# Ecogenomics/CheckM

Hardware: NVIDIA H100
Metric: genomes/hour (higher is better)
Workload: dtype int16 (SSV) / u8 (MSV) / int16 (Viterbi) / f32 (Forward, domain definition)

## Files before the change

checkm_b200/csrc/fwdback_blk.cuh:

```cuda
#pragma once
#include "device_utils.cuh"
#include "engine.hpp"
#include "fwdback.cuh"

namespace ckm {

constexpr int BLK_LOOKAHEAD_MAXQ = 16;

template <int Q, bool TSMEM>
struct BlkModel {
  int M;
  const float *rfb;
  const float4 *tsm;
  float4 t0[TSMEM ? 1 : Q], t1[TSMEM ? 1 : Q];
  int lane;
  __device__ __forceinline__ float4 T0(int q) const { return TSMEM ? tsm[q * 32 + lane] : t0[TSMEM ? 0 : q]; }
  __device__ __forceinline__ float4 T1(int q) const { return TSMEM ? tsm[(Q + q) * 32 + lane] : t1[TSMEM ? 0 : q]; }
};

template <int Q, bool TSMEM>
__device__ __forceinline__ void blk_model_load(BlkModel<Q, TSMEM> &bm, const ModelScalars &ms, const float4 *tfb, const float *rfb,
                                               float4 *tsm, int lane) {
  bm.M = ms.M; bm.lane = lane;
  bm.rfb = rfb + ms.blk_off * 32 * KPAD + lane;
  bm.tsm = tsm;
  const float4 *src = tfb + ms.blk_off * 32 * 2;
  if (TSMEM) {
    __syncwarp();
    for (int q = 0; q < Q; ++q) { tsm[q * 32 + lane] = __ldg(src + (q * 32 + lane) * 2); tsm[(Q + q) * 32 + lane] = __ldg(src + (q * 32 + lane) * 2 + 1); }
    __syncwarp();
  } else {
#pragma unroll
    for (int q = 0; q < Q; ++q) { bm.t0[TSMEM ? 0 : q] = __ldg(src + (q * 32 + lane) * 2); bm.t1[TSMEM ? 0 : q] = __ldg(src + (q * 32 + lane) * 2 + 1); }
  }
}

template <int Q, bool TSMEM, bool FULL, bool STORE_D = true>
__device__ __forceinline__ float forward_blk(const BlkModel<Q, TSMEM> &bm, const uint8_t *__restrict__ res, int L, const Specials sp,
                                             float *xmx, float *full) {
  const int lane = bm.lane;
  float Mx[Q], Ix[Q], Dx[Q];
#pragma unroll
  for (int q = 0; q < Q; ++q) { Mx[q] = 0.0f; Ix[q] = 0.0f; Dx[q] = 0.0f; }
  if (FULL) {
#pragma unroll
    for (int z = 0; z < 3 * Q; ++z) full[z * 32 + lane] = 0.0f;
  }
  float xE = 0.0f, xN = 1.0f, xJ = 0.0f, xB = sp.nmove, xC = 0.0f, totscale = 0.0f;
  if (xmx != nullptr && lane == 0) { xmx[X_E] = xE; xmx[X_N] = xN; xmx[X_J] = xJ; xmx[X_B] = xB; xmx[X_C] = xC; xmx[X_SCALE] = 1.0f; }
  constexpr bool LA = (Q <= BLK_LOOKAHEAD_MAXQ);
  float ecur[Q];
  int xnext;
  if (LA) {
    const float *rp = bm.rfb + (size_t)((L >= 1) ? __ldg(res) : 0) * Q * 32;
#pragma unroll
    for (int q = 0; q < Q; ++q) ecur[q] = __ldg(rp + q * 32);
    xnext = (L >= 2) ? __ldg(res + 1) : 0;
  } else xnext = (L >= 1) ? __ldg(res) : 0;
  for (int i = 1; i <= L; ++i) {
    float enext[LA ? Q : 1];
    {
      const float *rp = bm.rfb + (size_t)xnext * Q * 32;
      if (LA) {
#pragma unroll
        for (int q = 0; q < Q; ++q) enext[LA ? q : 0] = __ldg(rp + q * 32);
        xnext = (i + 2 <= L) ? __ldg(res + i + 1) : 0;
      } else {
#pragma unroll
        for (int q = 0; q < Q; ++q) ecur[q] = __ldg(rp + q * 32);
        xnext = (i + 1 <= L) ? __ldg(res + i) : 0;
      }
    }
    float pm_in = __shfl_up_sync(0xffffffffu, Mx[Q - 1], 1), pi_in = __shfl_up_sync(0xffffffffu, Ix[Q - 1], 1), pd_in = __shfl_up_sync(0xffffffffu, Dx[Q - 1], 1);
    if (lane == 0) { pm_in = 0.0f; pi_in = 0.0f; pd_in = 0.0f; }
    float md[Q], esum = 0.0f;
#pragma unroll
    for (int q = Q - 1; q >= 0; --q) {
      const float4 t0 = bm.T0(q), t1 = bm.T1(q);
      const float pm = (q > 0) ? Mx[q - 1] : pm_in, pi = (q > 0) ? Ix[q - 1] : pi_in, pd = (q > 0) ? Dx[q - 1] : pd_in;
      float sv = xB * t0.x;
      sv += pm * t0.y;
      sv += pi * t0.z;
      sv += pd * t0.w;
      sv *= ecur[q];
      const float nI = Mx[q] * t1.y + Ix[q] * t1.z;
      md[q] = sv * t1.x;
      Mx[q] = sv; Ix[q] = nI;
      esum += sv;
    }
    float Bb = 0.0f, Tb = 1.0f;
#pragma unroll
    for (int q = 0; q < Q; ++q) { const float tdd = bm.T1(q).w; Bb = md[q] + Bb * tdd; Tb *= tdd; }
    float Bs = Bb, Ts = Tb;
#pragma unroll
    for (int o = 1; o < 32; o <<= 1) {
      const float Bl = __shfl_up_sync(0xffffffffu, Bs, o), Tl = __shfl_up_sync(0xffffffffu, Ts, o);
      if (lane >= o) { Bs = Bs + Bl * Ts; Ts = Ts * Tl; }
    }
    float d = __shfl_up_sync(0xffffffffu, Bs, 1);
    if (lane == 0) d = 0.0f;
#pragma unroll
    for (int q = 0; q < Q; ++q) {
// ... 5 lines not shown
    xE = warp_sum_float(esum);
    xN = xN * sp.nloop;
    xC = (xC * sp.nloop) + (xE * sp.emove);
    xJ = (xJ * sp.nloop) + (xE * sp.eloop);
    xB = (xJ * sp.nmove) + (xN * sp.nmove);
    float scale = 1.0f;
    if (xE > 1.0e4f) {
      scale = xE;
      const float inv = __fdiv_rn(1.0f, xE);
      xN = __fdiv_rn(xN, xE); xC = __fdiv_rn(xC, xE); xJ = __fdiv_rn(xJ, xE); xB = __fdiv_rn(xB, xE);
#pragma unroll
      for (int q = 0; q < Q; ++q) { Mx[q] *= inv; Dx[q] *= inv; Ix[q] *= inv; }
      totscale += (float)log((double)xE);
      xE = 1.0f;
    }
    if (FULL) {
      float *fr = full + (size_t)i * 3 * Q * 32 + lane;
#pragma unroll
      for (int q = 0; q < Q; ++q) { fr[q * 32] = Mx[q]; if (STORE_D) fr[(Q + q) * 32] = Dx[q]; fr[(2 * Q + q) * 32] = Ix[q]; }
    }
    if (xmx != nullptr && lane == 0) {
      float *xr = xmx + (size_t)i * X_NX;
      xr[X_E] = xE; xr[X_N] = xN; xr[X_J] = xJ; xr[X_B] = xB; xr[X_C] = xC; xr[X_SCALE] = scale;
    }
    if (LA) {
#pragma unroll
      for (int q = 0; q < Q; ++q) ecur[q] = enext[LA ? q : 0];
    }
  }
  return totscale + (float)log((double)(xC * sp.nmove));
}

__device__ __forceinline__ void prefetch_l2(const void *p) { asm volatile("prefetch.global.L2 [%0];" ::"l"(p)); }
template <int Q, bool TSMEM, int MODE>
__device__ __forceinline__ void backward_blk(const BlkModel<Q, TSMEM> &bm, const uint8_t *__restrict__ res, int L, const Specials sp,
                                             const float *fxmx, float *bxmx, float *full) {
  const int lane = bm.lane, M = bm.M;
  float Mx[Q], Ix[Q], Dx[Q];
#pragma unroll
  for (int q = 0; q < Q; ++q) { Mx[q] = 0.0f; Ix[q] = 0.0f; Dx[q] = 0.0f; }
  float xC = 0.0f, xE = 0.0f, xJ = 0.0f, xN = 0.0f, xB = 0.0f;
  constexpr bool LA = (Q <= BLK_LOOKAHEAD_MAXQ);
  float ecur[Q];
#pragma unroll
  for (int q = 0; q < Q; ++q) ecur[q] = 0.0f;
  int xnext = (L >= 1) ? __ldg(res + L - 1) : 0;
  for (int i = L; i >= 0; --i) {
    float enext[LA ? Q : 1];
    if (LA) {
      const float *rp = bm.rfb + (size_t)xnext * Q * 32;
#pragma unroll
      for (int q = 0; q < Q; ++q) enext[LA ? q : 0] = __ldg(rp + q * 32);
      xnext = (i >= 2) ? __ldg(res + i - 2) : 0;
    } else if (i < L) {
      const float *rp = bm.rfb + (size_t)xnext * Q * 32;
#pragma unroll
      for (int q = 0; q < Q; ++q) ecur[q] = __ldg(rp + q * 32);
      xnext = (i >= 1) ? __ldg(res + i - 1) : 0;
    }
    if (MODE == 2 && i >= 3) {
      const float *fr = full + (size_t)(i - 2) * 3 * Q * 32;
      if (lane < Q) { prefetch_l2(fr + lane * 32); prefetch_l2(fr + (2 * Q + lane) * 32); }
    }
    float em[Q];
    if (i == L) {
      xC = sp.nmove; xE = xC * sp.emove; xB = 0.0f; xJ = 0.0f; xN = 0.0f;
#pragma unroll
      for (int q = 0; q < Q; ++q) em[q] = 0.0f;
    } else {
      float part = 0.0f;
#pragma unroll
      for (int q = 0; q < Q; ++q) { em[q] = Mx[q] * ecur[q]; part += em[q] * bm.T0(q).x; }
      xB = warp_sum_float(part);
      xC = xC * sp.nloop;
      xJ = (xB * sp.nmove) + (xJ * sp.nloop);
      xN = (xB * sp.nmove) + (xN * sp.nloop);
      xE = (xC * sp.emove) + (xJ * sp.eloop);
    }
    const float s = (i >= 1) ? fxmx[(size_t)i * X_NX + X_SCALE] : 1.0f;
    if (i >= 1) {
      const float inv = (s > 1.0f) ? __fdiv_rn(1.0f, s) : 1.0f;
      float em_next = __shfl_down_sync(0xffffffffu, em[0], 1);
      float4 tn_next;
      {
        const float4 mine = bm.T0(0);
        tn_next.x = 0.0f;
        tn_next.y = __shfl_down_sync(0xffffffffu, mine.y, 1); tn_next.z = __shfl_down_sync(0xffffffffu, mine.z, 1); tn_next.w = __shfl_down_sync(0xffffffffu, mine.w, 1);
      }
      if (lane == 31) { em_next = 0.0f; tn_next.y = 0.0f; tn_next.z = 0.0f; tn_next.w = 0.0f; }
      float cb[Q];
// ... 70 lines not shown
```

checkm_b200/csrc/kernels_blk.cu:

```cuda
#include "engine.hpp"
#include "device_utils.cuh"
#include "stages.hpp"
#include "fwdback.cuh"
#include "fwdback_blk.cuh"
#include "domdef_common.cuh"
#include "filter_common.cuh"

namespace ckm {

constexpr int BLK_WARPS = 4;

__host__ __device__ constexpr size_t blk_tsm_bytes(int Q) { return (size_t)Q * 32 * 2 * sizeof(float4); }

template <int Q, bool TSMEM>
__global__ void __launch_bounds__(BLK_WARPS * 32) fwd2_kernel(FilterParams p) {
  extern __shared__ __align__(16) uint8_t bsm[];
  const int lane = threadIdx.x & 31, warp = threadIdx.x >> 5;
  float4 *tsm = reinterpret_cast<float4 *>(bsm) + (size_t)warp * Q * 32 * 2;
  const int n = min(*p.in_count, p.in_cap);
  for (int c = blockIdx.x * BLK_WARPS + warp; c < n; c += gridDim.x * BLK_WARPS) {
    Candidate cd = p.in[c];
    const ModelScalars ms = p.ms[cd.model];
    if (ms.vq != Q) continue;
    const int s = cd.seq, L = p.len[s];
    BlkModel<Q, TSMEM> bm;
    blk_model_load<Q, TSMEM>(bm, ms, p.tfb, p.rfb, tsm, lane);
    const float fsc = forward_blk<Q, TSMEM, false>(bm, p.res + p.off[s], L, make_specials(L, true), nullptr, nullptr);
    fwd_verdict(p, cd, fsc, ms, lane);
  }
}

template <int Q, bool TSMEM>
__global__ void __launch_bounds__(BLK_WARPS * 32) regions2_kernel(DomdefParams p) {
  extern __shared__ __align__(16) uint8_t bsm[];
  const int lane = threadIdx.x & 31, warp = threadIdx.x >> 5;
  float4 *tsm = reinterpret_cast<float4 *>(bsm) + (size_t)warp * Q * 32 * 2;
  for (int idx = p.pair_begin + blockIdx.x * BLK_WARPS + warp; idx < p.pair_end; idx += gridDim.x * BLK_WARPS) {
    const int pi = p.pair_order[idx];
    const PairWork pw = p.pairs[pi];
    const ModelScalars ms = p.ms[pw.model];
    if (ms.vq != Q) continue;
    const int L = pw.L;
    BlkModel<Q, TSMEM> bm;
    blk_model_load<Q, TSMEM>(bm, ms, p.tfb, p.rfb, tsm, lane);
    const uint8_t *res = p.res + p.off[pw.seq];
    const Specials sp = make_specials(L, true);
    float *xf = p.xf + pw.row_off * X_NX, *xb = p.xb + pw.row_off * X_NX;
    forward_blk<Q, TSMEM, false>(bm, res, L, sp, xf, nullptr);
    __syncwarp();
    backward_blk<Q, TSMEM, 0>(bm, res, L, sp, xf, xb, nullptr);
    __syncwarp();
    regions_tail(p, pi, L, sp, xf, xb, p.btot + pw.row_off, p.etot + pw.row_off, p.mocc + pw.row_off, p.n2sc + pw.row_off, lane);
    __syncwarp();
  }
}

template <int Q> struct BlockedLayout {
  const float *F; const float4 *tfb; int M;
  static __device__ __forceinline__ int at(int k) { return ((k - 1) % Q) * 32 + (k - 1) / Q; }
  __device__ __forceinline__ float cell(int row, int plane, int k) const { return F[((int64_t)row * 3 + plane) * (Q * 32) + at(k)]; }
  __device__ __forceinline__ float4 t0(int k) const { return __ldg(tfb + at(k) * 2); }
// ... 144 lines not shown
          if (lane >= o && Ps) { As = fmaxf(As, Al); Ps = (pl != 0); }
        }
        float d = __shfl_up_sync(0xffffffffu, As, 1);
        if (lane == 0) d = NINF;
#pragma unroll
        for (int q = 0; q < Q; ++q) {
          const bool in = (lane * Q + q + 1) <= M;
          oD[q] = in ? d : NINF;
          emax = fmaxf(emax, oD[q]);
          d = ps[q] ? fmaxf(a[q], d) : a[q];
        }
#pragma unroll
        for (int o = 16; o > 0; o >>= 1) emax = fmaxf(emax, __shfl_xor_sync(0xffffffffu, emax, o));
        os.row(sp, pps + r * 3, emax);
#pragma unroll
        for (int q = 0; q < Q; ++q) { orow[q * 32] = oM[q]; orow[(Q + q) * 32] = oD[q]; orow[(2 * Q + q) * 32] = oI[q]; }
        os.store(xo + (int64_t)r * X_NX, lane);
      }
      oasc = os.C;
    }
    __syncwarp();
    OaTrace tr;
    if (!range_err) tr = oa_traceback(BlockedLayout<Q>{Bm, p.tfb + ms.blk_off * 64, M}, p, pw, env, sp, xo, pps, Ld, M, lane);
    write_domain(p, env, n2sc, tr, envsc, oasc, lane);
    __syncwarp();
  }
}

template <class P, class KF>
static int launch_blk(KF kern, const char *name, int Q, bool tsmem, const P &p, int grid, size_t extra, cudaStream_t st) {
  return launch_kernel(kern, name, grid, BLK_WARPS * 32, (tsmem ? BLK_WARPS * blk_tsm_bytes(Q) : 0) + extra, st, p);
}
int launch_fwd2(const FilterParams &p, int cls, int grid, cudaStream_t st) {
  return with_class(cls, [&](auto Q, auto TSMEM) { return launch_blk(fwd2_kernel<Q, TSMEM>, "fwd2_kernel", Q, TSMEM, p, grid, 0, st); });
}
int launch_regions2(const DomdefParams &p, int cls, int grid, cudaStream_t st) {
  return with_class(cls, [&](auto Q, auto TSMEM) { return launch_blk(regions2_kernel<Q, TSMEM>, "regions2_kernel", Q, TSMEM, p, grid, 0, st); });
}
int launch_envelopes2(const DomdefParams &p, int cls, int grid, cudaStream_t st) {
  return with_class(cls, [&](auto Q, auto TSMEM) {
    return launch_blk(envelope2_kernel<Q, TSMEM>, "envelope2_kernel", Q, TSMEM, p, grid, BLK_WARPS * 32 * sizeof(float), st);
  });
}

}
```

checkm_b200/csrc/kernels_vitp.cu:

```cuda
#include "engine.hpp"
#include "device_utils.cuh"
#include "stages.hpp"
#include "filter_common.cuh"

namespace ckm {

constexpr uint32_t VP_FLOORW = 0xD800D800u;
constexpr int      VP_FLOOR  = -10240;
constexpr uint32_t VP_TFLOORW = 0xC000C000u;

__device__ __forceinline__ int vp_lo(uint32_t w) { return (int)(int16_t)(w & 0xffffu); }
__device__ __forceinline__ int vp_hi(uint32_t w) { return (int)w >> 16; }

__global__ void vit_count_kernel(FilterParams p, int32_t *cnt) {
  const int n = min(*p.in_count, p.in_cap);
  for (int i = blockIdx.x * blockDim.x + threadIdx.x; i < n; i += gridDim.x * blockDim.x) {
    const Candidate cd = p.in[i];
    if (!(cd.P > p.F2)) filter_pass(p, cd, 4);
    else if (p.ms[cd.model].vq == 0) vit_redo(p, cd);
    else atomicAdd(cnt + cd.model, 1);
  }
}

__global__ void __launch_bounds__(1024) vit_scan_kernel(FilterParams p, int32_t nmodels, const int32_t *cnt, int32_t *off, int32_t *choff) {
  __shared__ int ws[2][32];
  const int lane = threadIdx.x & 31, warp = threadIdx.x >> 5;
  int run_pairs = 0, run_chunks = 0;
  for (int c = 0; c < N_BLK_CLASSES; ++c) {
    if (threadIdx.x == 0) p.vit_cls_chunks[c] = run_chunks;
    for (int b = 0; b < nmodels; b += 1024) {
      const int m = b + threadIdx.x;
      const int v = (m < nmodels && blk_class(p.ms[m].vq) == c) ? cnt[m] : 0, h = (v + VITP_CHUNK - 1) / VITP_CHUNK;
      int sv = v, sh = h;
#pragma unroll
      for (int o = 1; o < 32; o <<= 1) {
        const int a = __shfl_up_sync(0xffffffffu, sv, o), d = __shfl_up_sync(0xffffffffu, sh, o);
        if (lane >= o) { sv += a; sh += d; }
      }
      if (lane == 31) { ws[0][warp] = sv; ws[1][warp] = sh; }
      __syncthreads();
      if (warp == 0) {
        int tv = ws[0][lane], th = ws[1][lane];
#pragma unroll
        for (int o = 1; o < 32; o <<= 1) {
          const int a = __shfl_up_sync(0xffffffffu, tv, o), d = __shfl_up_sync(0xffffffffu, th, o);
          if (lane >= o) { tv += a; th += d; }
        }
        ws[0][lane] = tv; ws[1][lane] = th;
      }
      __syncthreads();
      if (v > 0) {
        off[m] = run_pairs + (warp ? ws[0][warp - 1] : 0) + sv - v;
        choff[m] = run_chunks + (warp ? ws[1][warp - 1] : 0) + sh - h;
      }
      run_pairs += ws[0][31]; run_chunks += ws[1][31];
      __syncthreads();
    }
  }
  if (threadIdx.x == 0) p.vit_cls_chunks[N_BLK_CLASSES] = run_chunks;
}

__global__ void vit_scatter_kernel(FilterParams p, const int32_t *cnt, int32_t *fill, const int32_t *off, const int32_t *choff) {
  const int n = min(*p.in_count, p.in_cap);
  for (int i = blockIdx.x * blockDim.x + threadIdx.x; i < n; i += gridDim.x * blockDim.x) {
    const int m = p.in[i].model;
    if (!(p.in[i].P > p.F2) || p.ms[m].vq == 0) continue;
    const int r = atomicAdd(fill + m, 1), pos = off[m] + r;
    p.vit_idx[pos] = i;
    if (r % VITP_CHUNK == 0) p.vit_chunks[choff[m] + r / VITP_CHUNK] = make_int2(pos, off[m] + min(r + VITP_CHUNK, cnt[m]));
  }
}

int launch_vit_group(const FilterParams &p, int32_t nmodels, int32_t *ws, int grid, cudaStream_t st) {
  int32_t *cnt = ws, *fill = ws + nmodels, *off = ws + 2 * (size_t)nmodels, *choff = ws + 3 * (size_t)nmodels;
  cudaError_t e = cudaMemsetAsync(ws, 0, sizeof(int32_t) * 2 * (size_t)nmodels, st);
  if (e != cudaSuccess) return cuda_fail(e, "cudaMemsetAsync(vit groups)");
  vit_count_kernel<<<grid, 256, 0, st>>>(p, cnt);
  vit_scan_kernel<<<1, 1024, 0, st>>>(p, nmodels, cnt, off, choff);
  vit_scatter_kernel<<<grid, 256, 0, st>>>(p, cnt, fill, off, choff);
  e = cudaGetLastError();
  return e == cudaSuccess ? CKM_OK : cuda_fail(e, "vit grouping launch");
}

constexpr int VITP_THREADS = 128;

__host__ __device__ constexpr int vitp_smem_bytes(int W, bool tsmem) { return KPAD * W * 32 * 4 + (tsmem ? W * 64 * 16 : 0); }
__host__ __device__ constexpr int vitp_min_blocks(int W) { return W <= 4 ? 4 : (W <= 10 ? 3 : 2); }

template <int W, bool TSMEM>
__global__ void __launch_bounds__(VITP_THREADS, vitp_min_blocks(W)) vitp_kernel(FilterParams p, int cls) {
  extern __shared__ __align__(16) uint4 vsm[];
  __shared__ int s_chunk, s_next;
  __shared__ ModelScalars s_ms;
  uint32_t *esm = reinterpret_cast<uint32_t *>(vsm);
  uint4 *tws = vsm + KPAD * W * 8;
  const int lane = threadIdx.x & 31;
  const uint32_t sel = (lane == 0) ? 0x1054u : 0x3210u;
  const int c0 = p.vit_cls_chunks[cls], nch = p.vit_cls_chunks[cls + 1] - c0;
  for (;;) {
    __syncthreads();
    if (threadIdx.x == 0) {
      const int k = atomicAdd(p.vit_work + cls, 1);
      s_chunk = k;
      if (k < nch) {
        s_next = p.vit_chunks[c0 + k].x;
        s_ms = p.ms[p.in[p.vit_idx[s_next]].model];
      }
    }
    __syncthreads();
    const int k = s_chunk;
    if (k >= nch) break;
    const int2 ch = p.vit_chunks[c0 + k];
    const ModelScalars &ms = s_ms;
    {
      const uint4 *esrc = reinterpret_cast<const uint4 *>(p.rwp + ms.blk_off * 32 * (KPAD / 2));
      for (int z = threadIdx.x; z < KPAD * W * 8; z += VITP_THREADS) vsm[z] = __ldg(esrc + z);
      if (TSMEM) {
        const uint4 *tsrc = p.twp + ms.blk_off * 32;
        for (int z = threadIdx.x; z < W * 64; z += VITP_THREADS) tws[(z & 1) * (W * 32) + (z >> 1)] = __ldg(tsrc + z);
      }
    }
    uint4 tr0[TSMEM ? 1 : W], tr1[TSMEM ? 1 : W];
    if (!TSMEM) {
      const uint4 *tsrc = p.twp + ms.blk_off * 32;
#pragma unroll
      for (int w = 0; w < W; ++w) { tr0[TSMEM ? 0 : w] = __ldg(tsrc + (w * 32 + lane) * 2); tr1[TSMEM ? 0 : w] = __ldg(tsrc + (w * 32 + lane) * 2 + 1); }
    }
#define TR0(w) (TSMEM ? tws[(w) * 32 + lane] : tr0[TSMEM ? 0 : (w)])
#define TR1(w) (TSMEM ? tws[W * 32 + (w) * 32 + lane] : tr1[TSMEM ? 0 : (w)])
    __syncthreads();
    const uint32_t *erow = esm + lane;
    const int ddbound = ms.ddbound_w, cap = 32767 - (int)ms.vit_emax;
    const int e_move = ms.xw_e_move, e_loop = ms.xw_e_loop;
    for (;;) {
      int j = 0;
      if (lane == 0) j = atomicAdd(&s_next, 1);
      j = __shfl_sync(0xffffffffu, j, 0);
      if (j >= ch.y) break;
      const Candidate *cin = p.in + p.vit_idx[j];
      const int s = cin->seq, L = p.len[s];
      bool redo = false;
      const int tmove = p.tmove_w[s];
      const int cost = -tmove - (int)ms.vit_tbm + 64;
      const bool c1 = (cost - (int)ms.xw_e_loop <= 22528) && (cost <= 22240);
      const bool c1p = (cost - (int)ms.xw_e_loop <= 16384);
      redo = !c1;
      float vsc = 0.0f;
      if (!redo) {
        uint32_t Mx[W], Ix[W], Dx[W];
#pragma unroll
        for (int w = 0; w < W; ++w) { Mx[w] = VP_FLOORW; Ix[w] = VP_FLOORW; Dx[w] = VP_FLOORW; }
        int xN = ms.base_w, xB = xN + tmove, xJ = -32768, xC = -32768;
        const uint32_t *rp = reinterpret_cast<const uint32_t *>(p.res + p.off[s]);
        const int nw = (L + 3) >> 2;
        uint32_t wcur = (nw > 0) ? __ldg(rp) : 0u;
        bool stop = false;
        for (int q = 0; q < nw && !stop; ++q) {
          const uint32_t wnext = (q + 1 < nw) ? __ldg(rp + q + 1) : 0u;
#pragma unroll
          for (int rr = 0; rr < 4; ++rr) {
            if (q * 4 + rr >= L) { stop = true; break; }
            const uint32_t *ew = erow + ((wcur >> (8 * rr)) & 0xffu) * (W * 32);
            const uint32_t shM = __shfl_sync(0xffffffffu, Mx[W - 1], (lane + 31) & 31);
            const uint32_t shI = __shfl_sync(0xffffffffu, Ix[W - 1], (lane + 31) & 31);
            const uint32_t shD = __shfl_sync(0xffffffffu, Dx[W - 1], (lane + 31) & 31);
            const uint32_t pm0 = __byte_perm(shM, VP_FLOORW, sel), pi0 = __byte_perm(shI, VP_FLOORW, sel), pd0 = __byte_perm(shD, VP_FLOORW, sel);
            const uint32_t xBw = __byte_perm((uint32_t)xB, 0u, 0x1010u);
            uint32_t md[W];
            uint32_t xEw = VP_FLOORW, dmw = VP_FLOORW;
#pragma unroll
            for (int w = W - 1; w >= 0; --w) {
              const uint32_t pm = (w > 0) ? Mx[w - 1] : pm0, pi = (w > 0) ? Ix[w - 1] : pi0, pd = (w > 0) ? Dx[w - 1] : pd0;
// ... 83 lines not shown
```

checkm_b200/csrc/search.cu:

```cuda
#include <algorithm>
#include <atomic>
#include <chrono>
#include <cstdio>
#include <cmath>
#include <cstdlib>
#include <cstring>
#include <memory>
#include <vector>
#include "engine.hpp"
#include "stages.hpp"
#include "pool.hpp"

using namespace ckm;

namespace ckm {

std::atomic<int> g_live_engines{0};
thread_local ckm_engine *g_pool_engine = nullptr;
thread_local int g_pool_next = 0;
constexpr int X_NX_HOST = 6;
struct EnsembleJob;
int ensembles_launch(ckm_engine *e, const ckm_models *m, DomdefParams &p, const std::vector<PairWork> &pairs,
                     const std::vector<Region> &regs, const std::vector<int> &multi_idx, const std::vector<EnsembleCaps> &caps,
                     cudaStream_t st, EnsembleJob **job_out);
// ... 224 lines not shown
  for (int c = 0; c < 4; ++c) {
    if (gl[c].empty() || db->nseq == 0) continue;
    sp.group_list = s1.glist.as<int32_t>() + goff[c]; sp.ngroups = (int32_t)gl[c].size();
    sp.unit_counter = e->d_counters + CTR_UNIT4 + c;
    int64_t maxbytes = 0;
    for (int g : gl[c]) maxbytes = std::max<int64_t>(maxbytes, m->groups[g].table_bytes);
    const int64_t units = (int64_t)sp.ngroups * sp.nchunks;
    const int grid = (int)std::min<int64_t>(nsm, units);
    if ((rc = launch_ssv(Js[c], sp, grid, (size_t)maxbytes, st))) return rc;
    e->stats.kernel_launches++;
  }
  if (!m->ssv_bypass.empty()) {
    if ((rc = launch_ssv_bypass(m->d_ssv_bypass, (int32_t)m->ssv_bypass.size(), db->nseq, db->d_len, db->d_bin,
                                am.all_active ? nullptr : am.model_active.as<uint8_t>(), (int32_t)m->models.size(),
                                s1.cand.as<int2>(), e->d_counters + CTR_CAND, s1.cand_cap, st))) return rc;
    e->stats.kernel_launches++;
  }
  CKM_CUDA(cudaEventRecord(e->ev[EV_MSV], st));
  MsvParams p{};
  p.res = db->d_res; p.off = db->d_off; p.len = db->d_len; p.nullsc = db->d_nullsc; p.tjb = db->d_tjb;
  p.ms = m->d_scalars; p.rbv = m->d_rbv; p.rmb = m->d_rmb;
  p.cand = s1.cand.as<int2>(); p.cand_count = e->d_counters + CTR_CAND; p.cand_cap = s1.cand_cap;
  p.out = s1.pass.as<Candidate>(); p.out_count = e->d_counters + CTR_MSV; p.out_cap = s1.pass_cap;
  p.xj_dense = xj_dense; p.model_slot = am.model_slot.as<int32_t>(); p.nseq = db->nseq;
  p.row_bytes = (m->maxM + 2 + 15) / 16 * 16;
  p.F1 = 0.02;
  p.use_blk = k.blk ? 1 : 0;
  if ((rc = per_class(e, p, launch_msv2, 16, launch_msv_exact, 4))) return rc;
  e->stats.kernel_launches += 1 + (p.use_blk ? N_BLK_CLASSES : 0);
  CKM_CUDA(cudaEventRecord(e->ev[EV_BIAS], st));
  return CKM_OK;
}

static int run_viterbi(ckm_engine *e, const ckm_models *m, FilterParams &p, bool packed, DevBuf &grp) {
  int rc;
  if (packed) {
    const int nm = (int)m->models.size();
    const size_t nchunks = (size_t)p.in_cap / VITP_CHUNK + nm + 1;
    const size_t words = 4 * (size_t)nm + 16 + ((size_t)p.in_cap + 1) / 2 * 2;
    if ((rc = grp.alloc(sizeof(int32_t) * words + sizeof(int2) * nchunks))) return rc;
    int32_t *ws = grp.as<int32_t>();
    p.vit_cls_chunks = ws + 4 * (size_t)nm;
    p.vit_idx = p.vit_cls_chunks + 16;
    p.vit_chunks = reinterpret_cast<int2 *>(ws + words);
    p.vit_work = e->d_counters + CTR_VWORK;
    if ((rc = launch_vit_group(p, nm, ws, e->prop.multiProcessorCount * 8, e->stream))) return rc;
    if ((rc = per_class<FilterParams>(e, p, launch_vitp, 8, nullptr, 0))) return rc;
    e->stats.kernel_launches += 3;
    p.in = p.redo; p.in_count = p.redo_count; p.in_cap = p.redo_cap;
  }
  return per_class(e, p, launch_vit2, 8, launch_vit, 4);
}
struct Stage2 {
  DevBuf a, b, redo, vgrp;
  int32_t cap = 0;
};
static int run_stage2(ckm_engine *e, const SearchKnobs &k, const ckm_models *m, const ckm_seqdb *db, ActiveMasks &am, Stage1 &s1, Stage2 &s2,
                      float *d_filtersc, float *d_vit, float *d_fwd, uint8_t *d_passed) {
  cudaStream_t st = e->stream;
  int rc;
  s2.cap = s1.pass_cap;
  if ((rc = s2.a.alloc(sizeof(Candidate) * (size_t)s2.cap))) return rc;
  if ((rc = s2.b.alloc(sizeof(Candidate) * (size_t)s2.cap))) return rc;
  if ((rc = s2.redo.alloc(sizeof(Candidate) * (size_t)s2.cap))) return rc;
  const int nsm = e->prop.multiProcessorCount;
  FilterParams p = filter_params(m, db, am);
  p.redo = s2.redo.as<Candidate>(); p.redo_count = e->d_counters + CTR_VREDO; p.redo_cap = s2.cap;
  p.use_blk = k.blk ? 1 : 0;
  p.dense_filtersc = d_filtersc; p.dense_vit = d_vit; p.dense_fwd = d_fwd; p.dense_passed = d_passed;
  p.in = s1.pass.as<Candidate>(); p.in_count = e->d_counters + CTR_MSV; p.in_cap = s1.pass_cap;
  p.out = s2.a.as<Candidate>(); p.out_count = e->d_counters + CTR_BIAS; p.out_cap = s2.cap;
  if ((rc = launch_bias(p, nsm * 8, st))) return rc;
  CKM_CUDA(cudaEventRecord(e->ev[EV_VIT], st));
  p.in = s2.a.as<Candidate>(); p.in_count = e->d_counters + CTR_BIAS; p.in_cap = s2.cap;
  p.out = s2.b.as<Candidate>(); p.out_count = e->d_counters + CTR_VIT; p.out_cap = s2.cap;
  if ((rc = run_viterbi(e, m, p, k.vitp, s2.vgrp))) return rc;
  CKM_CUDA(cudaEventRecord(e->ev[EV_FWD], st));
  p.in = s2.b.as<Candidate>(); p.in_count = e->d_counters + CTR_VIT; p.in_cap = s2.cap;
  p.out = s2.a.as<Candidate>(); p.out_count = e->d_counters + CTR_FWD; p.out_cap = s2.cap;
  if ((rc = per_class(e, p, launch_fwd2, 8, launch_fwd, 4, true))) return rc;
  CKM_CUDA(cudaEventRecord(e->ev[EV_CASCADE_END], st));
  e->stats.kernel_launches += 3 + (k.vitp ? N_BLK_CLASSES : 0) + (p.use_blk ? 2 * N_BLK_CLASSES : 0);
  return CKM_OK;
}

static int64_t envelope_need(const ckm_models *m, const PairWork &pw, const Envelope &en, bool use_blk) {
  const int64_t Ld = en.j - en.i + 1, Mpad = ((m->models[pw.model].M + 1) + 31) / 32 * 32 + 32;
  const int64_t vq = use_blk ? vq_of(m->models[pw.model].M) : 0;
  const int64_t width = vq ? 32 * vq : Mpad;
  return (vq ? 1 : 2) * (Ld + 1) * 3 * width + (Ld + 1) * 15 + 64;
}
static int run_envelope_waves(ckm_engine *e, const ckm_models *m, const std::vector<PairWork> &pairs, DomdefParams &p, int64_t budget,
                              DevBuf &scratch, std::vector<Envelope> &ev, DevBuf &d_ev, DevBuf &d_ord, bool leave_last) {
  if (ev.empty()) return CKM_OK;
  cudaStream_t st = e->stream;
  int rc;
  std::vector<int64_t> need(ev.size());
  std::vector<int8_t> ecls(ev.size());
  for (size_t i = 0; i < ev.size(); ++i) {
    const PairWork &pw = pairs[ev[i].pair];
    need[i] = envelope_need(m, pw, ev[i], p.use_blk != 0);
    ecls[i] = (int8_t)cls_of(m->models[pw.model].M, p.use_blk != 0);
  }
  budget = std::max<int64_t>(budget, *std::max_element(need.begin(), need.end()));
  if ((rc = d_ev.alloc(sizeof(Envelope) * ev.size())) || (rc = d_ord.alloc(sizeof(int32_t) * ev.size()))) return rc;
  std::vector<int32_t> eorder(ev.size());
  for (size_t w0 = 0, w1; w0 < ev.size(); w0 = w1) {
    int64_t tot = 0;
    for (w1 = w0; w1 < ev.size() && (w1 == w0 || tot + need[w1] <= budget); ++w1) { ev[w1].scratch_off = tot; tot += need[w1]; }
    if (sizeof(float) * (size_t)tot > scratch.bytes && (rc = scratch.alloc(sizeof(float) * (size_t)tot))) return rc;
    for (size_t i = w0; i < w1; ++i) eorder[i] = (int32_t)i;
    std::stable_sort(eorder.begin() + w0, eorder.begin() + w1, [&](int32_t a, int32_t b) { return ecls[a] != ecls[b] ? ecls[a] > ecls[b] : need[a] > need[b]; });
    CKM_CUDA(cudaMemcpyAsync(d_ev.as<Envelope>() + w0, ev.data() + w0, sizeof(Envelope) * (w1 - w0), cudaMemcpyHostToDevice, st));
    CKM_CUDA(cudaMemcpyAsync(d_ord.as<int32_t>() + w0, eorder.data() + w0, sizeof(int32_t) * (w1 - w0), cudaMemcpyHostToDevice, st));
    p.envs = d_ev.as<Envelope>(); p.env_order = d_ord.as<int32_t>(); p.scratch = scratch.as<float>();
// ... 532 lines not shown
```

checkm_b200/csrc/stages.hpp:

```cpp
#pragma once
#include <type_traits>
#include "engine.hpp"

namespace ckm {

#ifndef CKM_SSV_WARPS
#define CKM_SSV_WARPS 16
#endif
constexpr int SSV_WARPS = CKM_SSV_WARPS;
constexpr int SSV_WARPS_HOST = SSV_WARPS;
constexpr int MSV_WARPS = 8;

struct SsvParams {
  const uint8_t *res; const int64_t *off; const int32_t *len; const int32_t *bin;
  const float *msvB; const int32_t *tjb; const int32_t *order;
  int32_t nseq, seq_chunk, nchunks;
  const TileGroup *groups; const int32_t *group_list; int32_t ngroups;
  const TileDesc *tiles; const TileModel *tile_models;
  const int32_t *chain_first_tile, *chain_ntiles;
  const uint8_t *tile_blob;
  const uint8_t *tile_active;
  const uint8_t *model_active;
  int32_t ntiles, nmodels;
  int32_t *unit_counter;
  int2 *cand; int32_t *cand_count; int32_t cand_cap;
  int16_t *bnd; int64_t bnd_stride;
  unsigned long long *cells;
  int32_t resolve;
  const ModelScalars *ms; const float *nullsc;
  Candidate *pass; int32_t *pass_count; int32_t pass_cap;
  int32_t *resolved_count;
  int32_t *xj_dense; const int32_t *model_slot;
  double F1;
};

int launch_ssv(int J, const SsvParams &p, int grid, size_t smem_bytes, cudaStream_t stream);

struct MsvParams {
  const uint8_t *res; const int64_t *off; const int32_t *len;
  const float *nullsc; const int32_t *tjb;
  const ModelScalars *ms; const uint8_t *rbv; const uint32_t *rmb;
  const int2 *cand; const int32_t *cand_count; int32_t cand_cap;
  Candidate *out; int32_t *out_count; int32_t out_cap;
  int32_t *xj_dense;
  const int32_t *model_slot;
  int32_t nseq;
  int32_t row_bytes;
  int32_t use_blk;
  double F1;
};

int launch_msv_exact(const MsvParams &p, int grid, cudaStream_t stream);
int launch_ssv_bypass(const int32_t *models, int32_t nbypass, int32_t nseq, const int32_t *len, const int32_t *bin,
                      const uint8_t *model_active, int32_t nmodels_db, int2 *cand, int32_t *cand_count, int32_t cand_cap,
                      cudaStream_t stream);
int launch_msv2(const MsvParams &p, int cls, int grid, cudaStream_t stream);

constexpr int VIT_WARPS = 4;
constexpr int FWD_WARPS = 4;
struct FilterParams {
  const uint8_t *res; const int64_t *off; const int32_t *len;
  const float *lenA, *lenB;
  const int16_t *tmove_w;
  const ModelScalars *ms;
  const float *bias_eo; const int16_t *rwv; const int16_t *twv; const float *rfv; const float *tfv;
  const uint4 *twb; const uint32_t *rwb; const float4 *tfb; const float *rfb;
  const uint4 *twp; const uint32_t *rwp;
  Candidate *redo; int32_t *redo_count; int32_t redo_cap;
  int32_t *vit_idx; int2 *vit_chunks; int32_t *vit_cls_chunks; int32_t *vit_work;
  const Candidate *in; const int32_t *in_count; int32_t in_cap;
  Candidate *out; int32_t *out_count; int32_t out_cap;
  int32_t row_elems;
  double F1, F2, F3;
  int32_t use_blk;
  float *dense_filtersc, *dense_vit, *dense_fwd; uint8_t *dense_passed;
  const int32_t *model_slot; int32_t nseq;
};
int launch_bias(const FilterParams &p, int grid, cudaStream_t st);
int launch_vit(const FilterParams &p, int grid, cudaStream_t st);
constexpr int N_BLK_CLASSES = 10;
constexpr int BLK_Q[N_BLK_CLASSES] = {2, 4, 6, 8, 12, 16, 20, 24, 28, 32};
constexpr bool blk_tsmem(int q) { return q >= 12; }
__host__ __device__ constexpr int vq_of(int M) { return M <= 256 ? 2 * ((M + 63) / 64) : M <= 1024 ? 4 * ((M + 127) / 128) : 0; }
__host__ __device__ constexpr int blk_class(int vq) { return vq == 0 ? N_BLK_CLASSES : (vq <= 8 ? vq / 2 - 1 : vq / 4 + 1); }
constexpr bool blk_table_ok(int c = 0) {
  return c == N_BLK_CLASSES || (blk_class(BLK_Q[c]) == c && vq_of(32 * BLK_Q[c]) == BLK_Q[c] &&
                                vq_of(32 * BLK_Q[c] + 1) == (c + 1 < N_BLK_CLASSES ? BLK_Q[c + 1] : 0) && blk_table_ok(c + 1));
}
static_assert(vq_of(1) == 2 && blk_table_ok(), "lane-block class arithmetic disagrees with BLK_Q");

template <int C = 0, class F> int with_class(int cls, F &&f) {
  if constexpr (C == N_BLK_CLASSES) {
    set_error("bad lane-block class " + std::to_string(cls));
    return CKM_EINVAL;
  } else {
    if (cls == C) return f(std::integral_constant<int, BLK_Q[C]>{}, std::integral_constant<bool, blk_tsmem(BLK_Q[C])>{});
    return with_class<C + 1>(cls, f);
  }
}

template <class... KA, class... A>
int launch_kernel(void (*kern)(KA...), const char *name, int grid, int block, size_t smem, cudaStream_t st, const A &...args) {
  cudaError_t e;
  if (smem > 48 * 1024 && (e = cudaFuncSetAttribute(kern, cudaFuncAttributeMaxDynamicSharedMemorySize, (int)smem)) != cudaSuccess)
    return cuda_fail(e, name);
  kern<<<grid, block, smem, st>>>(args...);
  e = cudaGetLastError();
  return e == cudaSuccess ? CKM_OK : cuda_fail(e, name);
}

int launch_vit2(const FilterParams &p, int cls, int grid, cudaStream_t st);
int launch_vitp(const FilterParams &p, int cls, int grid, cudaStream_t st);
constexpr int VITP_CHUNK = 64;
int launch_vit_group(const FilterParams &p, int32_t nmodels, int32_t *ws, int grid, cudaStream_t st);
int launch_all_pairs(Candidate *out, int32_t *count, const int32_t *slot_model, int32_t nslots, int32_t nseq, cudaStream_t st);
int launch_fwd(const FilterParams &p, int grid, cudaStream_t st);

#define FLT_MIN_F 1.17549435e-38f
struct PairWork {
  int32_t seq, model, L;
  int32_t first_dom, ndom_slots;
  float   fwdsc, filtersc, usc;
  int64_t row_off;
};
struct Region { int32_t pair, i, j, multi; };
constexpr int ENS_MAXENV = 32;
struct EnsembleCaps { int32_t segments, trace_segments, envelopes; };
constexpr EnsembleCaps ENS_DEFAULT_CAPS = {4096, 64, ENS_MAXENV};
struct Envelope { int32_t pair, i, j, null2_done; int64_t scratch_off; int32_t slot, pad; };
struct DomainOut {
  int32_t pair, ienv, jenv, hmmfrom, hmmto, sqfrom, sqto, ok;
  float   envsc, domcorrection, oasc, bitscore, dombias, pad;
  double  lnP;
};
struct HitOut { float pre_score, score, sum_score; int32_t ndom, valid, pad; double lnP; };
struct DomdefParams {
  const uint8_t *res; const int64_t *off; const float *nullsc;
  const ModelScalars *ms; const float *rfv; const float *tfv;
  const PairWork *pairs; int32_t npairs;
  const int32_t *pair_order; int32_t pair_begin, pair_end;
  float *xf, *xb, *btot, *etot, *mocc, *n2sc;
  int32_t *trace;
  Region *regions; int32_t *region_count; int32_t region_cap;
  const Envelope *envs; const int32_t *env_order; int32_t env_begin, env_end;
  float *scratch;
  DomainOut *doms; HitOut *hits;
  const float *logsum_tbl;
// ... 13 lines not shown
```

Before: 35390.

## Group forward-filter candidates by model and stage emissions in shared memory

```diff
diff --git a/checkm_b200/csrc/fwdback_blk.cuh b/checkm_b200/csrc/fwdback_blk.cuh
--- a/checkm_b200/csrc/fwdback_blk.cuh
+++ b/checkm_b200/csrc/fwdback_blk.cuh
@@ -7,7 +7,7 @@
 
 constexpr int BLK_LOOKAHEAD_MAXQ = 16;
 
-template <int Q, bool TSMEM>
+template <int Q, bool TSMEM, bool ESMEM = false>
 struct BlkModel {
   int M;
   const float *rfb;
@@ -16,6 +16,7 @@
   int lane;
   __device__ __forceinline__ float4 T0(int q) const { return TSMEM ? tsm[q * 32 + lane] : t0[TSMEM ? 0 : q]; }
   __device__ __forceinline__ float4 T1(int q) const { return TSMEM ? tsm[(Q + q) * 32 + lane] : t1[TSMEM ? 0 : q]; }
+  __device__ __forceinline__ float E(const float *p) const { if constexpr (ESMEM) return *p; else return __ldg(p); }
 };
 
 template <int Q, bool TSMEM>
@@ -35,8 +36,8 @@
   }
 }
 
-template <int Q, bool TSMEM, bool FULL, bool STORE_D = true>
-__device__ __forceinline__ float forward_blk(const BlkModel<Q, TSMEM> &bm, const uint8_t *__restrict__ res, int L, const Specials sp,
+template <int Q, bool TSMEM, bool FULL, bool STORE_D = true, bool ESMEM = false>
+__device__ __forceinline__ float forward_blk(const BlkModel<Q, TSMEM, ESMEM> &bm, const uint8_t *__restrict__ res, int L, const Specials sp,
                                              float *xmx, float *full) {
   const int lane = bm.lane;
   float Mx[Q], Ix[Q], Dx[Q];
@@ -48,13 +49,13 @@
   }
   float xE = 0.0f, xN = 1.0f, xJ = 0.0f, xB = sp.nmove, xC = 0.0f, totscale = 0.0f;
   if (xmx != nullptr && lane == 0) { xmx[X_E] = xE; xmx[X_N] = xN; xmx[X_J] = xJ; xmx[X_B] = xB; xmx[X_C] = xC; xmx[X_SCALE] = 1.0f; }
-  constexpr bool LA = (Q <= BLK_LOOKAHEAD_MAXQ);
+  constexpr bool LA = !ESMEM && Q <= BLK_LOOKAHEAD_MAXQ;
   float ecur[Q];
   int xnext;
   if (LA) {
     const float *rp = bm.rfb + (size_t)((L >= 1) ? __ldg(res) : 0) * Q * 32;
 #pragma unroll
-    for (int q = 0; q < Q; ++q) ecur[q] = __ldg(rp + q * 32);
+    for (int q = 0; q < Q; ++q) ecur[q] = bm.E(rp + q * 32);
     xnext = (L >= 2) ? __ldg(res + 1) : 0;
   } else xnext = (L >= 1) ? __ldg(res) : 0;
   for (int i = 1; i <= L; ++i) {
@@ -63,11 +64,11 @@
       const float *rp = bm.rfb + (size_t)xnext * Q * 32;
       if (LA) {
 #pragma unroll
-        for (int q = 0; q < Q; ++q) enext[LA ? q : 0] = __ldg(rp + q * 32);
+        for (int q = 0; q < Q; ++q) enext[LA ? q : 0] = bm.E(rp + q * 32);
         xnext = (i + 2 <= L) ? __ldg(res + i + 1) : 0;
       } else {
 #pragma unroll
-        for (int q = 0; q < Q; ++q) ecur[q] = __ldg(rp + q * 32);
+        for (int q = 0; q < Q; ++q) ecur[q] = bm.E(rp + q * 32);
         xnext = (i + 1 <= L) ? __ldg(res + i) : 0;
       }
     }
@@ -139,15 +140,15 @@
 }
 
 __device__ __forceinline__ void prefetch_l2(const void *p) { asm volatile("prefetch.global.L2 [%0];" ::"l"(p)); }
-template <int Q, bool TSMEM, int MODE>
-__device__ __forceinline__ void backward_blk(const BlkModel<Q, TSMEM> &bm, const uint8_t *__restrict__ res, int L, const Specials sp,
+template <int Q, bool TSMEM, int MODE, bool ESMEM = false>
+__device__ __forceinline__ void backward_blk(const BlkModel<Q, TSMEM, ESMEM> &bm, const uint8_t *__restrict__ res, int L, const Specials sp,
                                              const float *fxmx, float *bxmx, float *full) {
   const int lane = bm.lane, M = bm.M;
   float Mx[Q], Ix[Q], Dx[Q];
 #pragma unroll
   for (int q = 0; q < Q; ++q) { Mx[q] = 0.0f; Ix[q] = 0.0f; Dx[q] = 0.0f; }
   float xC = 0.0f, xE = 0.0f, xJ = 0.0f, xN = 0.0f, xB = 0.0f;
-  constexpr bool LA = (Q <= BLK_LOOKAHEAD_MAXQ);
+  constexpr bool LA = !ESMEM && Q <= BLK_LOOKAHEAD_MAXQ;
   float ecur[Q];
 #pragma unroll
   for (int q = 0; q < Q; ++q) ecur[q] = 0.0f;
@@ -157,12 +158,12 @@
     if (LA) {
       const float *rp = bm.rfb + (size_t)xnext * Q * 32;
 #pragma unroll
-      for (int q = 0; q < Q; ++q) enext[LA ? q : 0] = __ldg(rp + q * 32);
+      for (int q = 0; q < Q; ++q) enext[LA ? q : 0] = bm.E(rp + q * 32);
       xnext = (i >= 2) ? __ldg(res + i - 2) : 0;
     } else if (i < L) {
       const float *rp = bm.rfb + (size_t)xnext * Q * 32;
 #pragma unroll
-      for (int q = 0; q < Q; ++q) ecur[q] = __ldg(rp + q * 32);
+      for (int q = 0; q < Q; ++q) ecur[q] = bm.E(rp + q * 32);
       xnext = (i >= 1) ? __ldg(res + i - 1) : 0;
     }
     if (MODE == 2 && i >= 3) {
diff --git a/checkm_b200/csrc/kernels_blk.cu b/checkm_b200/csrc/kernels_blk.cu
--- a/checkm_b200/csrc/kernels_blk.cu
+++ b/checkm_b200/csrc/kernels_blk.cu
@@ -12,21 +12,60 @@
 
 __host__ __device__ constexpr size_t blk_tsm_bytes(int Q) { return (size_t)Q * 32 * 2 * sizeof(float4); }
 
+__host__ __device__ constexpr bool fwd2_esmem(int Q) { return Q <= 20; }
+__host__ __device__ constexpr size_t fwd2_smem_bytes(int Q, bool tsmem) {
+  return (tsmem ? blk_tsm_bytes(Q) : 0) + (fwd2_esmem(Q) ? (size_t)KPAD * Q * 32 * sizeof(float) : 0);
+}
+__host__ __device__ constexpr int fwd2_min_blocks(int Q) { return Q <= 4 ? 4 : (Q <= 12 ? 3 : 2); }
+
 template <int Q, bool TSMEM>
-__global__ void __launch_bounds__(BLK_WARPS * 32) fwd2_kernel(FilterParams p) {
+__global__ void __launch_bounds__(BLK_WARPS * 32, fwd2_min_blocks(Q)) fwd2_kernel(FilterParams p, int cls) {
+  constexpr bool ESMEM = fwd2_esmem(Q);
   extern __shared__ __align__(16) uint8_t bsm[];
-  const int lane = threadIdx.x & 31, warp = threadIdx.x >> 5;
-  float4 *tsm = reinterpret_cast<float4 *>(bsm) + (size_t)warp * Q * 32 * 2;
-  const int n = min(*p.in_count, p.in_cap);
-  for (int c = blockIdx.x * BLK_WARPS + warp; c < n; c += gridDim.x * BLK_WARPS) {
-    Candidate cd = p.in[c];
-    const ModelScalars ms = p.ms[cd.model];
-    if (ms.vq != Q) continue;
-    const int s = cd.seq, L = p.len[s];
-    BlkModel<Q, TSMEM> bm;
-    blk_model_load<Q, TSMEM>(bm, ms, p.tfb, p.rfb, tsm, lane);
-    const float fsc = forward_blk<Q, TSMEM, false>(bm, p.res + p.off[s], L, make_specials(L, true), nullptr, nullptr);
-    fwd_verdict(p, cd, fsc, ms, lane);
+  __shared__ int s_next, s_end;
+  __shared__ ModelScalars s_ms;
+  float4 *tsm = reinterpret_cast<float4 *>(bsm);
+  float *esm = reinterpret_cast<float *>(bsm + (TSMEM ? blk_tsm_bytes(Q) : 0));
+  const int lane = threadIdx.x & 31;
+  for (;;) {
+    __syncthreads();
+    if (threadIdx.x == 0) {
+      const int c0 = p.grp.cls_chunks[cls], k = atomicAdd(p.grp.work + cls, 1);
+      s_end = -1;
+      if (k < p.grp.cls_chunks[cls + 1] - c0) {
+        const int2 ch = p.grp.chunks[c0 + k];
+        s_next = ch.x; s_end = ch.y;
+        s_ms = p.ms[p.in[p.grp.idx[ch.x]].model];
+      }
+    }
+    __syncthreads();
+    if (s_end < 0) break;
+    const ModelScalars &ms = s_ms;
+    {
+      const float4 *tsrc = p.tfb + ms.blk_off * 32 * 2;
+      if (TSMEM) for (int z = threadIdx.x; z < Q * 64; z += blockDim.x) tsm[(z & 1) * (Q * 32) + (z >> 1)] = __ldg(tsrc + z);
+      const float4 *esrc = reinterpret_cast<const float4 *>(p.rfb + ms.blk_off * 32 * KPAD);
+      if (ESMEM) for (int z = threadIdx.x; z < KPAD * Q * 8; z += blockDim.x) reinterpret_cast<float4 *>(esm)[z] = __ldg(esrc + z);
+    }
+    BlkModel<Q, TSMEM, ESMEM> bm;
+    bm.M = ms.M; bm.lane = lane; bm.tsm = tsm;
+    bm.rfb = (ESMEM ? esm : p.rfb + ms.blk_off * 32 * KPAD) + lane;
+    if (!TSMEM) {
+      const float4 *src = p.tfb + ms.blk_off * 32 * 2;
+#pragma unroll
+      for (int q = 0; q < Q; ++q) { bm.t0[TSMEM ? 0 : q] = __ldg(src + (q * 32 + lane) * 2); bm.t1[TSMEM ? 0 : q] = __ldg(src + (q * 32 + lane) * 2 + 1); }
+    }
+    __syncthreads();
+    for (;;) {
+      int j = 0;
+      if (lane == 0) j = atomicAdd(&s_next, 1);
+      j = __shfl_sync(0xffffffffu, j, 0);
+      if (j >= s_end) break;
+      Candidate cd = p.in[p.grp.idx[j]];
+      const int s = cd.seq, L = p.len[s];
+      const float fsc = forward_blk<Q, TSMEM, false>(bm, p.res + p.off[s], L, make_specials(L, true), nullptr, nullptr);
+      fwd_verdict(p, cd, fsc, ms, lane);
+    }
   }
 }
 
@@ -237,7 +276,9 @@
   return launch_kernel(kern, name, grid, BLK_WARPS * 32, (tsmem ? BLK_WARPS * blk_tsm_bytes(Q) : 0) + extra, st, p);
 }
 int launch_fwd2(const FilterParams &p, int cls, int grid, cudaStream_t st) {
-  return with_class(cls, [&](auto Q, auto TSMEM) { return launch_blk(fwd2_kernel<Q, TSMEM>, "fwd2_kernel", Q, TSMEM, p, grid, 0, st); });
+  return with_class(cls, [&](auto Q, auto TSMEM) {
+    return launch_kernel(fwd2_kernel<Q, TSMEM>, "fwd2_kernel", grid, BLK_WARPS * 32, fwd2_smem_bytes(Q, TSMEM), st, p, cls);
+  });
 }
 int launch_regions2(const DomdefParams &p, int cls, int grid, cudaStream_t st) {
   return with_class(cls, [&](auto Q, auto TSMEM) { return launch_blk(regions2_kernel<Q, TSMEM>, "regions2_kernel", Q, TSMEM, p, grid, 0, st); });
diff --git a/checkm_b200/csrc/kernels_vitp.cu b/checkm_b200/csrc/kernels_vitp.cu
--- a/checkm_b200/csrc/kernels_vitp.cu
+++ b/checkm_b200/csrc/kernels_vitp.cu
@@ -12,25 +12,28 @@
 __device__ __forceinline__ int vp_lo(uint32_t w) { return (int)(int16_t)(w & 0xffffu); }
 __device__ __forceinline__ int vp_hi(uint32_t w) { return (int)w >> 16; }
 
-__global__ void vit_count_kernel(FilterParams p, int32_t *cnt) {
+__device__ __forceinline__ bool group_skip(const FilterParams &p, const Candidate &cd, bool viterbi) {
+  return (viterbi && !(cd.P > p.F2)) || p.ms[cd.model].vq == 0;
+}
+__global__ void group_count_kernel(FilterParams p, int32_t *cnt, bool viterbi) {
   const int n = min(*p.in_count, p.in_cap);
   for (int i = blockIdx.x * blockDim.x + threadIdx.x; i < n; i += gridDim.x * blockDim.x) {
     const Candidate cd = p.in[i];
-    if (!(cd.P > p.F2)) filter_pass(p, cd, 4);
-    else if (p.ms[cd.model].vq == 0) vit_redo(p, cd);
+    if (viterbi && !(cd.P > p.F2)) filter_pass(p, cd, 4);
+    else if (p.ms[cd.model].vq == 0) { if (viterbi) vit_redo(p, cd); }
     else atomicAdd(cnt + cd.model, 1);
   }
 }
 
-__global__ void __launch_bounds__(1024) vit_scan_kernel(FilterParams p, int32_t nmodels, const int32_t *cnt, int32_t *off, int32_t *choff) {
+__global__ void __launch_bounds__(1024) group_scan_kernel(FilterParams p, int32_t nmodels, const int32_t *cnt, int32_t *off, int32_t *choff, int chunk) {
   __shared__ int ws[2][32];
   const int lane = threadIdx.x & 31, warp = threadIdx.x >> 5;
   int run_pairs = 0, run_chunks = 0;
   for (int c = 0; c < N_BLK_CLASSES; ++c) {
-    if (threadIdx.x == 0) p.vit_cls_chunks[c] = run_chunks;
+    if (threadIdx.x == 0) p.grp.cls_chunks[c] = run_chunks;
     for (int b = 0; b < nmodels; b += 1024) {
       const int m = b + threadIdx.x;
-      const int v = (m < nmodels && blk_class(p.ms[m].vq) == c) ? cnt[m] : 0, h = (v + VITP_CHUNK - 1) / VITP_CHUNK;
+      const int v = (m < nmodels && blk_class(p.ms[m].vq) == c) ? cnt[m] : 0, h = (v + chunk - 1) / chunk;
       int sv = v, sh = h;
 #pragma unroll
       for (int o = 1; o < 32; o <<= 1) {
@@ -57,29 +60,29 @@
       __syncthreads();
     }
   }
-  if (threadIdx.x == 0) p.vit_cls_chunks[N_BLK_CLASSES] = run_chunks;
-}
-
-__global__ void vit_scatter_kernel(FilterParams p, const int32_t *cnt, int32_t *fill, const int32_t *off, const int32_t *choff) {
+  if (threadIdx.x == 0) p.grp.cls_chunks[N_BLK_CLASSES] = run_chunks;
+}
+
+__global__ void group_scatter_kernel(FilterParams p, const int32_t *cnt, int32_t *fill, const int32_t *off, const int32_t *choff, int chunk, bool viterbi) {
   const int n = min(*p.in_count, p.in_cap);
   for (int i = blockIdx.x * blockDim.x + threadIdx.x; i < n; i += gridDim.x * blockDim.x) {
+    if (group_skip(p, p.in[i], viterbi)) continue;
     const int m = p.in[i].model;
-    if (!(p.in[i].P > p.F2) || p.ms[m].vq == 0) continue;
     const int r = atomicAdd(fill + m, 1), pos = off[m] + r;
-    p.vit_idx[pos] = i;
-    if (r % VITP_CHUNK == 0) p.vit_chunks[choff[m] + r / VITP_CHUNK] = make_int2(pos, off[m] + min(r + VITP_CHUNK, cnt[m]));
-  }
-}
-
-int launch_vit_group(const FilterParams &p, int32_t nmodels, int32_t *ws, int grid, cudaStream_t st) {
+    p.grp.idx[pos] = i;
+    if (r % chunk == 0) p.grp.chunks[choff[m] + r / chunk] = make_int2(pos, off[m] + min(r + chunk, cnt[m]));
+  }
+}
+
+int launch_group(const FilterParams &p, int32_t nmodels, int32_t *ws, int chunk, bool viterbi, int grid, cudaStream_t st) {
   int32_t *cnt = ws, *fill = ws + nmodels, *off = ws + 2 * (size_t)nmodels, *choff = ws + 3 * (size_t)nmodels;
   cudaError_t e = cudaMemsetAsync(ws, 0, sizeof(int32_t) * 2 * (size_t)nmodels, st);
-  if (e != cudaSuccess) return cuda_fail(e, "cudaMemsetAsync(vit groups)");
-  vit_count_kernel<<<grid, 256, 0, st>>>(p, cnt);
-  vit_scan_kernel<<<1, 1024, 0, st>>>(p, nmodels, cnt, off, choff);
-  vit_scatter_kernel<<<grid, 256, 0, st>>>(p, cnt, fill, off, choff);
+  if (e != cudaSuccess) return cuda_fail(e, "cudaMemsetAsync(model groups)");
+  group_count_kernel<<<grid, 256, 0, st>>>(p, cnt, viterbi);
+  group_scan_kernel<<<1, 1024, 0, st>>>(p, nmodels, cnt, off, choff, chunk);
+  group_scatter_kernel<<<grid, 256, 0, st>>>(p, cnt, fill, off, choff, chunk, viterbi);
   e = cudaGetLastError();
-  return e == cudaSuccess ? CKM_OK : cuda_fail(e, "vit grouping launch");
+  return e == cudaSuccess ? CKM_OK : cuda_fail(e, "model grouping launch");
 }
 
 constexpr int VITP_THREADS = 128;
@@ -96,21 +99,21 @@
   uint4 *tws = vsm + KPAD * W * 8;
   const int lane = threadIdx.x & 31;
   const uint32_t sel = (lane == 0) ? 0x1054u : 0x3210u;
-  const int c0 = p.vit_cls_chunks[cls], nch = p.vit_cls_chunks[cls + 1] - c0;
+  const int c0 = p.grp.cls_chunks[cls], nch = p.grp.cls_chunks[cls + 1] - c0;
   for (;;) {
     __syncthreads();
     if (threadIdx.x == 0) {
-      const int k = atomicAdd(p.vit_work + cls, 1);
+      const int k = atomicAdd(p.grp.work + cls, 1);
       s_chunk = k;
       if (k < nch) {
-        s_next = p.vit_chunks[c0 + k].x;
-        s_ms = p.ms[p.in[p.vit_idx[s_next]].model];
+        s_next = p.grp.chunks[c0 + k].x;
+        s_ms = p.ms[p.in[p.grp.idx[s_next]].model];
       }
     }
     __syncthreads();
     const int k = s_chunk;
     if (k >= nch) break;
-    const int2 ch = p.vit_chunks[c0 + k];
+    const int2 ch = p.grp.chunks[c0 + k];
     const ModelScalars &ms = s_ms;
     {
       const uint4 *esrc = reinterpret_cast<const uint4 *>(p.rwp + ms.blk_off * 32 * (KPAD / 2));
@@ -137,7 +140,7 @@
       if (lane == 0) j = atomicAdd(&s_next, 1);
       j = __shfl_sync(0xffffffffu, j, 0);
       if (j >= ch.y) break;
-      const Candidate *cin = p.in + p.vit_idx[j];
+      const Candidate *cin = p.in + p.grp.idx[j];
       const int s = cin->seq, L = p.len[s];
       bool redo = false;
       const int tmove = p.tmove_w[s];
diff --git a/checkm_b200/csrc/search.cu b/checkm_b200/csrc/search.cu
--- a/checkm_b200/csrc/search.cu
+++ b/checkm_b200/csrc/search.cu
@@ -280,19 +280,24 @@
   return CKM_OK;
 }
 
+static int group_pairs(ckm_engine *e, const ckm_models *m, FilterParams &p, DevBuf &grp, int chunk, bool viterbi) {
+  const int nm = (int)m->models.size();
+  const size_t nchunks = (size_t)p.in_cap / FWD2_CHUNK + nm + 1;
+  const size_t words = 4 * (size_t)nm + 16 + ((size_t)p.in_cap + 1) / 2 * 2;
+  int rc;
+  if ((rc = grp.alloc(sizeof(int32_t) * words + sizeof(int2) * nchunks))) return rc;
+  int32_t *ws = grp.as<int32_t>();
+  p.grp.cls_chunks = ws + 4 * (size_t)nm;
+  p.grp.idx = p.grp.cls_chunks + 16;
+  p.grp.chunks = reinterpret_cast<int2 *>(ws + words);
+  p.grp.work = e->d_counters + CTR_VWORK;
+  CKM_CUDA(cudaMemsetAsync(p.grp.work, 0, sizeof(int32_t) * N_BLK_CLASSES, e->stream));
+  return launch_group(p, nm, ws, chunk, viterbi, e->prop.multiProcessorCount * 8, e->stream);
+}
 static int run_viterbi(ckm_engine *e, const ckm_models *m, FilterParams &p, bool packed, DevBuf &grp) {
   int rc;
   if (packed) {
-    const int nm = (int)m->models.size();
-    const size_t nchunks = (size_t)p.in_cap / VITP_CHUNK + nm + 1;
-    const size_t words = 4 * (size_t)nm + 16 + ((size_t)p.in_cap + 1) / 2 * 2;
-    if ((rc = grp.alloc(sizeof(int32_t) * words + sizeof(int2) * nchunks))) return rc;
-    int32_t *ws = grp.as<int32_t>();
-    p.vit_cls_chunks = ws + 4 * (size_t)nm;
-    p.vit_idx = p.vit_cls_chunks + 16;
-    p.vit_chunks = reinterpret_cast<int2 *>(ws + words);
-    p.vit_work = e->d_counters + CTR_VWORK;
-    if ((rc = launch_vit_group(p, nm, ws, e->prop.multiProcessorCount * 8, e->stream))) return rc;
+    if ((rc = group_pairs(e, m, p, grp, VITP_CHUNK, true))) return rc;
     if ((rc = per_class<FilterParams>(e, p, launch_vitp, 8, nullptr, 0))) return rc;
     e->stats.kernel_launches += 3;
     p.in = p.redo; p.in_count = p.redo_count; p.in_cap = p.redo_cap;
@@ -300,7 +305,7 @@
   return per_class(e, p, launch_vit2, 8, launch_vit, 4);
 }
 struct Stage2 {
-  DevBuf a, b, redo, vgrp;
+  DevBuf a, b, redo, grp;
   int32_t cap = 0;
 };
 static int run_stage2(ckm_engine *e, const SearchKnobs &k, const ckm_models *m, const ckm_seqdb *db, ActiveMasks &am, Stage1 &s1, Stage2 &s2,
@@ -322,13 +327,14 @@
   CKM_CUDA(cudaEventRecord(e->ev[EV_VIT], st));
   p.in = s2.a.as<Candidate>(); p.in_count = e->d_counters + CTR_BIAS; p.in_cap = s2.cap;
   p.out = s2.b.as<Candidate>(); p.out_count = e->d_counters + CTR_VIT; p.out_cap = s2.cap;
-  if ((rc = run_viterbi(e, m, p, k.vitp, s2.vgrp))) return rc;
+  if ((rc = run_viterbi(e, m, p, k.vitp, s2.grp))) return rc;
   CKM_CUDA(cudaEventRecord(e->ev[EV_FWD], st));
   p.in = s2.b.as<Candidate>(); p.in_count = e->d_counters + CTR_VIT; p.in_cap = s2.cap;
   p.out = s2.a.as<Candidate>(); p.out_count = e->d_counters + CTR_FWD; p.out_cap = s2.cap;
+  if (p.use_blk && (rc = group_pairs(e, m, p, s2.grp, FWD2_CHUNK, false))) return rc;
   if ((rc = per_class(e, p, launch_fwd2, 8, launch_fwd, 4, true))) return rc;
   CKM_CUDA(cudaEventRecord(e->ev[EV_CASCADE_END], st));
-  e->stats.kernel_launches += 3 + (k.vitp ? N_BLK_CLASSES : 0) + (p.use_blk ? 2 * N_BLK_CLASSES : 0);
+  e->stats.kernel_launches += 3 + (k.vitp ? N_BLK_CLASSES : 0) + (p.use_blk ? 2 * N_BLK_CLASSES + 3 : 0);
   return CKM_OK;
 }
 
diff --git a/checkm_b200/csrc/stages.hpp b/checkm_b200/csrc/stages.hpp
--- a/checkm_b200/csrc/stages.hpp
+++ b/checkm_b200/csrc/stages.hpp
@@ -56,6 +56,7 @@
                       cudaStream_t stream);
 int launch_msv2(const MsvParams &p, int cls, int grid, cudaStream_t stream);
 
+struct ModelGroups { int32_t *idx; int2 *chunks; int32_t *cls_chunks; int32_t *work; };
 constexpr int VIT_WARPS = 4;
 constexpr int FWD_WARPS = 4;
 struct FilterParams {
@@ -67,7 +68,7 @@
   const uint4 *twb; const uint32_t *rwb; const float4 *tfb; const float *rfb;
   const uint4 *twp; const uint32_t *rwp;
   Candidate *redo; int32_t *redo_count; int32_t redo_cap;
-  int32_t *vit_idx; int2 *vit_chunks; int32_t *vit_cls_chunks; int32_t *vit_work;
+  ModelGroups grp;
   const Candidate *in; const int32_t *in_count; int32_t in_cap;
   Candidate *out; int32_t *out_count; int32_t out_cap;
   int32_t row_elems;
@@ -112,7 +113,8 @@
 int launch_vit2(const FilterParams &p, int cls, int grid, cudaStream_t st);
 int launch_vitp(const FilterParams &p, int cls, int grid, cudaStream_t st);
 constexpr int VITP_CHUNK = 64;
-int launch_vit_group(const FilterParams &p, int32_t nmodels, int32_t *ws, int grid, cudaStream_t st);
+constexpr int FWD2_CHUNK = 16;
+int launch_group(const FilterParams &p, int32_t nmodels, int32_t *ws, int chunk, bool viterbi, int grid, cudaStream_t st);
 int launch_all_pairs(Candidate *out, int32_t *count, const int32_t *slot_model, int32_t nslots, int32_t nseq, cudaStream_t st);
 int launch_fwd(const FilterParams &p, int grid, cudaStream_t st);
 
```

Measured after the change: 35670, median of 6. No clear change (+0.8%).
